# LouisBearing/BirdSoundClassif

Hardware: AMD Instinct MI355X
Metric: clips/sec (3 s @ 22.05 kHz) detect fwd (higher is better)
Workload: dtype f32; 1 GPU; BASELINE.json configs[1]: 1xMI355X inference, batch=64 synthetic 3 s clips (PCM16 @22.05 kHz resident in HBM) through the HIP STFT front end + detector forward + device post-processing, detections returned to the host; batch_per_gpu=64, distinct_clips=64, lanes=2

## Files before the change

birdsoundclassif_amd/_lib.py:

```python
import ctypes as C
import os
import subprocess

_HERE = os.path.dirname(os.path.abspath(__file__))
LIB_PATH = os.environ.get('NBM_LIB') or os.path.join(_HERE, 'libnbm_hip.so')
CSRC = os.path.join(_HERE, 'csrc')

_lib = None


class GemmDesc(C.Structure):
    _fields_ = [('x', C.c_void_p), ('w', C.c_void_p), ('y', C.c_void_p),
                ('scale', C.c_void_p), ('shift', C.c_void_p), ('residual', C.c_void_p),
                ('x_gs', C.c_int64), ('w_gs', C.c_int64), ('y_gs', C.c_int64), ('res_gs', C.c_int64),
                ('groups', C.c_int),
                ('B', C.c_int), ('H', C.c_int), ('W', C.c_int), ('Cin', C.c_int),
                ('N', C.c_int),
                ('kh', C.c_int), ('kw', C.c_int), ('stride', C.c_int), ('pad', C.c_int),
                ('Ho', C.c_int), ('Wo', C.c_int),
                ('x_ld', C.c_int), ('w_ld', C.c_int), ('y_ld', C.c_int), ('res_ld', C.c_int),
                ('alpha', C.c_float), ('act', C.c_int), ('shift_per_row', C.c_int),
                ('up', C.c_void_p), ('up_H', C.c_int), ('up_W', C.c_int),
                ('rows', C.c_void_p), ('rows_blocks', C.c_void_p),
                ('rows_mode', C.c_int), ('rows_count', C.c_int), ('rows_TH', C.c_int), ('rows_TW', C.c_int),
                ('mask', C.c_void_p), ('mask_ld', C.c_int), ('bits_out', C.c_void_p)]


class RoiDesc(C.Structure):
    _fields_ = [('fmap', C.c_void_p * 5), ('fh', C.c_int * 5), ('fw', C.c_int * 5),
                ('n_levels', C.c_int), ('C', C.c_int),
                ('rois', C.c_void_p), ('n_roi', C.c_void_p), ('B', C.c_int), ('roi_cap', C.c_int),
                ('pe_f', C.c_void_p), ('pe_t', C.c_void_p), ('img_h', C.c_int), ('img_w', C.c_int),
                ('pool', C.c_void_p), ('pe', C.c_void_p), ('level', C.c_void_p)]


class AugmentParams(C.Structure):
    _fields_ = [('gain', C.c_float), ('coef', C.c_float), ('denom', C.c_float), ('neg_coef', C.c_float),
                ('neg_denom', C.c_float), ('flags', C.c_int32), ('hard_index', C.c_int32), ('pad', C.c_int32),
                ('noise_seed', C.c_uint64)]


class BwdDesc(C.Structure):
    _fields_ = [('g', C.c_void_p), ('w', C.c_void_p), ('x', C.c_void_p), ('out', C.c_void_p),
                ('a_scale', C.c_void_p), ('row_scale', C.c_void_p), ('residual', C.c_void_p), ('mask', C.c_void_p),
                ('g_gs', C.c_int64), ('w_gs', C.c_int64), ('x_gs', C.c_int64), ('out_gs', C.c_int64), ('res_gs', C.c_int64),
                ('groups', C.c_int),
                ('B', C.c_int), ('H', C.c_int), ('W', C.c_int), ('Cin', C.c_int), ('N', C.c_int),
                ('kh', C.c_int), ('kw', C.c_int), ('stride', C.c_int), ('pad', C.c_int), ('Ho', C.c_int), ('Wo', C.c_int),
                ('g_ld', C.c_int), ('w_ld', C.c_int), ('x_ld', C.c_int), ('out_ld', C.c_int), ('res_ld', C.c_int),
                ('mask_ld', C.c_int), ('alpha', C.c_float), ('bias_grad', C.c_void_p), ('residual2', C.c_void_p), ('res2_ld', C.c_int),
                ('mask_bits', C.c_void_p)]


_P, _I, _L, _F, _U64 = C.c_void_p, C.c_int, C.c_int64, C.c_float, C.c_uint64

SIGNATURES = {
    'nbm_graph_census': [_P, C.POINTER(C.c_longlong * 6)],
    'nbm_copy_rect': [_P, _P, _L, _L, _I, _L, _L, _I, _I, _P],
    'nbm_gemm_conv': [C.POINTER(GemmDesc), _P],
    'nbm_pcm16_to_wave': [_P, _L, _I, _I, _I, _P, _L, _L, _P, _L, _I, _I, _P],
    'nbm_resample_to_wave': [_P, _L, _I, _L, _I, _I, _P, _I, _L, _L, _P, _L, _I, _I, _I, _P],
    'nbm_wav_decode': [_P, _L, _I, _I, _I, _I, _L, _P, _L, _P],
    'nbm_minmax_init': [_P, _I, _P],
    'nbm_stft_db': [_P, _L, _I, _I, _I, _I, _P, _I, _I, _I, _F, _P, _L, _I, _P, _P],
    'nbm_spec_windows': [_P, _L, _I, _I, _I, _I, _P, _P, _I, _I, _I, _P, _P],
    'nbm_spec_windows_table': [_P, _I, _I, _P, _I, _I, _P],
    'nbm_init_conv': [_P, _L, _P, _P, _I, _P, _P],
    'nbm_stem7x7': [_P, _I, _I, _I, _P, _P, _P, _P, _P, _P, _P],
    'nbm_stem7x7_wgrad': [_P, _P, _I, _I, _I, _P, _P, _P],
    'nbm_maxpool3x3s2': [_P, _I, _I, _I, _I, _P, _I, _I, _P, _P],
    'nbm_space_to_batch2': [_P, _I, _I, _I, _I, _P, _I, _P],
    'nbm_avgpool2x2': [_P, _I, _I, _I, _I, _P, _P],
    'nbm_avgpool2x2_bwd': [_P, _I, _I, _I, _I, _P, _P],
    'nbm_upsample_bilinear_add': [_P, _I, _I, _I, _I, _P, _P, _I, _I, _P],
    'nbm_softmax_rows': [_P, _L, _I, _L, _P],
    'nbm_dwconv3x3': [_P, _I, _I, _I, _I, _I, _I, _P, _P, _P, _L, _P, _I, _I, _P],
    'nbm_silu': [_P, _P, _L, _P],
    'nbm_layernorm': [_P, _L, _I, _P, _P, _F, _P, _P],
    'nbm_mha_small': [_P, _P, _P, _I, _I, _I, _P, _I, _I, _I, _I, _I, _L, _L, _P, _F, _P],
    'nbm_mha_segments': [_P, _P, _P, _I, _I, _I, _P, _I, _I, _I, _I, _I, _I, _P, _P, _I, _F, _P],
    'nbm_pair_softmax': [_P, _L, _I, _I, _P, _I, _P],
    'nbm_rpn_decode': [_P, _P, _P, _I, _I, _I, _I, _I, _I, _P, _P, _P, _P],
    'nbm_nan_images': [_P, _I, _L, _P, _P],
    'nbm_rpn_select': [_P, _P, _P, _I, _I, _I, _I, _I, _P, _P, _P, _P, _P],
    'nbm_nms_batched': [_P, _P, _P, _I, _I, _F, _I, _P, _P, _P, _P, _P, _P, _P],
    'nbm_roi_pool': [C.POINTER(RoiDesc), _P],
    'nbm_rcnn_post': [_P, _P, _I, _I, _P, _P, _I, _I, _I, _F, _F, _I, _P, _P, _P],
    'nbm_merge_collect': [_P, _P, _I, _I, _I, _I, _I, _L, _P, _P, _P, _P, _P, _P],
    'nbm_merge_nms_workspace': [_I, C.POINTER(C.c_int64)],
    'nbm_merge_nms': [_P, _P, _I, _F, _P, _L, _P, _P, _P],
    'nbm_merge_gather': [_P, _P, _P, _P, _P, _I, _P, _P, _P],
    'nbm_conv_dgrad': [C.POINTER(BwdDesc), _P],
    'nbm_conv_wgrad': [C.POINTER(BwdDesc), _P],
    'nbm_relu_bwd': [_P, _P, _P, _L, _P],
    'nbm_silu_bwd': [_P, _P, _P, _L, _P],
    'nbm_axpby': [_P, _P, _P, _F, _F, _L, _L, _P],
    'nbm_colsum': [_P, _L, _I, _I, _P, _P],
    'nbm_leaky_relu_bwd': [_P, _P, _P, _F, _L, _P],
    'nbm_layernorm_bwd': [_P, _P, _P, _L, _I, _F, _P, _P, _P, _P],
    'nbm_mha_small_bwd': [_P, _P, _P, _P, _I, _I, _I, _I, _P, _P, _P, _I, _I, _I, _P, _I, _I, _I, _I, _L, _L, _P, _F, _P],
    'nbm_zero_roi_windows': [_P, _I, _I, _I, _P, _P, _I, _I, _I, _P],
    'nbm_zero_pattern': [_P, _I, _I, _I, _I, _I, _P],
    'nbm_zero_tiles': [_P, _I, _I, _I, _I, _P, _I, _P, _P],
    'nbm_tiles_gather': [_P, _I, _I, _I, _I, _P, _I, _P, _P, _P],
    'nbm_tiles_scatter_add': [_P, _I, _I, _I, _I, _P, _I, _P, _P, _P],
    'nbm_proposal_iou': [_P, _P, _P, _I, _I, _I, _P, _P, _P],
    'nbm_anchor_targets': [_P, _I, _P, _P, _I, _I, _F, _F, _P, _P, _P, _P],
    'nbm_maxpool3x3s2_bwd': [_P, _P, _P, _I, _I, _I, _I, _I, _I, _P, _P, _P],
    'nbm_upsample_bilinear_bwd': [_P, _I, _I, _I, _I, _P, _I, _I, _I, _P],
    'nbm_tiles_upsample_bilinear_bwd_add': [_P, _I, _I, _I, _I, _P, _I, _P, _P, _I, _I, _P],
    'nbm_png_unfilter_gray8': [_P, _L, _I, _I, _I, _P, _L, _P, _P],
    'nbm_image_half_std_u8': [_P, _L, _I, _L, _P, _P],
    'nbm_randn_fill': [_U64, _L, _P, _P],
    'nbm_augment_batch': [_P, _P, _P, _I, _I, _I, _P, _P, _P, _P, _P, _P, _P],
    'nbm_u8_to_unit': [_P, _L, _P, _P],
    'nbm_wino_input': [_P, _I, _I, _I, _I, _P, _I, _P],
    'nbm_wino_output': [_P, _P, _P, _P, _I, _I, _I, _I, _I, _P, _I, _P, _P],
    'nbm_wino_outgrad': [_P, _I, _I, _I, _I, _P, _P, _I, _P],
    'nbm_wino_weight': [_P, _P, _I, _I, _I, _I, _P, _P],
    'nbm_wino_weight_grad': [_P, _P, _I, _I, _I, _P, _P],
    'nbm_wino23_rows': [_P, _I, _I, _I, _I, _P, _P],
    'nbm_wino23_conv_fused': [_P, _P, _P, _P, _P, _I, _I, _I, _I, _I, _I, _P, _I, _P],
    'nbm_wino23_rows_tiles': [_P, _I, _I, _I, _I, _P, _I, _P, _P, _P, _I, _P],
    'nbm_wino23_conv_fused_tiles': [_P, _P, _P, _P, _P, _I, _I, _I, _I, _I, _I, _P, _P, _I, _P, _P, _P],
    'nbm_roi_tiles': [_P, _P, _I, _I, _I, _I, _P, _P, _P, _I, _P, _P, _P],
    'nbm_wino23_input_tiles': [_P, _I, _I, _I, _I, _P, _I, _P, _P, _P],
    'nbm_wino23_outgrad_tiles': [_P, _I, _I, _I, _I, _P, _I, _P, _P, _P, _I, _P],
    'nbm_cell_outgrad': [_P, _I, _I, _I, _I, _I, _P, _P, _P],
    'nbm_cell_weight': [_P, _I, _I, _P, _I, _P, _I, _P],
    'nbm_cell_weight_fold': [_P, _P, _I, _I, _I, _I, _F, _P, _I, _P, _I, _P],
    'nbm_cell_weight_grad': [_P, _I, _I, _I, _P, _P],
    'nbm_cell_input': [_P, _I, _I, _I, _I, _I, _P, _I, _I, _P],
    'nbm_cell_input_up': [_P, _P, _I, _I, _I, _I, _I, _I, _I, _P, _I, _I, _P],
    'nbm_cell_patches': [_P, _I, _I, _I, _I, _I, _P, _I, _I, _P],
    'nbm_cell_patches_up': [_P, _P, _I, _I, _I, _I, _I, _I, _I, _P, _I, _I, _P],
    'nbm_cell_dgrad_output': [_P, _I, _I, _I, _I, _I, _P, _I, _I, _I, _P, _P],
    'nbm_cell_output': [_P, _P, _I, _I, _I, _I, _I, _P, _P],
    'nbm_weighted_sum': [_P, _P, _P, _P, _P, _L, _P],
    'nbm_weighted_sum_bwd': [_P, _P, _P, _P, _P, _P, _P, _P, _P, _L, _P],
    'nbm_softmax_rows_bwd': [_P, _P, _P, _L, _I, _F, _P],
    'nbm_pair_softmax_bwd': [_P, _P, _P, _L, _P],
    'nbm_dwconv3x3_bwd': [_P, _P, _P, _I, _I, _I, _I, _I, _I, _P, _P, _P, _I, _I, _P],
# ... 51 lines not shown
```

birdsoundclassif_amd/csrc/igemm.hip:

```cpp
#include <stdlib.h>
#include "nbm_common.h"
#include "igemm_params.h"
#include <type_traits>

namespace {

constexpr int BK = 32;
constexpr int PITCH = 36;

enum { A_FAST = 0, A_GENERIC = 1 };
enum { EPI_STD = 0 };

using nbm_igemm::IgemmParams;

template <int BM, int BN, int WM, int WN, int AMODE, int EPI, int STAGES = 2, bool ROWS = false>
__global__ __launch_bounds__(256, BM > 128 ? 1 : STAGES == 1 ? 3 : 2) void igemm_kernel(const IgemmParams p) {
  constexpr int MT = WM / 32, NT = WN / 32;
  constexpr int WAVES_N = BN / WN;
  constexpr int AR = BM / 32, BR = BN / 32;
  static_assert((BM / WM) * (BN / WN) == 4, "4 waves per workgroup");

  __shared__ __attribute__((aligned(16))) float lds[STAGES * (BM + BN) * PITCH];
  if constexpr (STAGES == 2) nbm_stagger_priority();
  float* As = lds;
// ... 319 lines not shown
#pragma unroll
        for (int j = 0; j < NTG; ++j) {
          const float* wb = Ws + ((g * NTG + j) * 32 + li) * WP + 16 * lh;
#pragma unroll
          for (int kc = 0; kc < K32; ++kc) {
            f32x4 b[4];
#pragma unroll
            for (int q = 0; q < 4; ++q) b[q] = *reinterpret_cast<const f32x4*>(wb + kc * 32 + 4 * q);
#pragma unroll
            for (int q = 0; q < 4; ++q)
#pragma unroll
              for (int e = 0; e < 4; ++e) acc[j] = __builtin_amdgcn_mfma_f32_32x32x2f32(a[kc][q][e], b[q][e], acc[j], 0, 0, 0);
          }
        }
      }
#pragma unroll
      for (int j = 0; j < NTG; ++j) {
        const int jj = g * NTG + j;
        __builtin_amdgcn_fence(__ATOMIC_ACQ_REL, "wavefront");
#pragma unroll
        for (int e = 0; e < 16; ++e) stg[((e & 3) + 8 * (e >> 2) + 4 * lh) * SPITCH + li] = acc[j][e];
        __builtin_amdgcn_fence(__ATOMIC_ACQ_REL, "wavefront");
        const int n = n_off + jj * 32 + ec;
        f32x4 sc = {1.f, 1.f, 1.f, 1.f}, sh = {0.f, 0.f, 0.f, 0.f};
        if (p.scale) sc = *reinterpret_cast<const f32x4*>(p.scale + n);
        if (p.shift) sh = *reinterpret_cast<const f32x4*>(p.shift + n);
#pragma unroll
        for (int pass = 0; pass < 4; ++pass) {
          const int r = pass * 8 + er, m = m0 + r;
          if (m >= p.M) continue;
          f32x4 v = *reinterpret_cast<const f32x4*>(stg + r * SPITCH + ec);
#pragma unroll
          for (int e = 0; e < 4; ++e) v[e] = (v[e] * p.alpha) * sc[e] + sh[e] + 0.f;
          if (p.residual) { v[0] += rq[j][pass][0]; v[1] += rq[j][pass][1]; v[2] += rq[j][pass][2]; v[3] += rq[j][pass][3]; }
          if (p.act == NBM_ACT_RELU) {
#pragma unroll
            for (int e = 0; e < 4; ++e) v[e] = fmaxf(v[e], 0.0f);
          } else if (p.act == NBM_ACT_SILU) {
#pragma unroll
            for (int e = 0; e < 4; ++e) v[e] = v[e] / (1.0f + expf(-v[e]));
          } else if (p.act == NBM_ACT_LEAKY) {
#pragma unroll
            for (int e = 0; e < 4; ++e) v[e] = v[e] > 0.f ? v[e] : 0.01f * v[e];
          }
          if (p.bits_out) {
            const int grp8 = 8 * er;
            const unsigned wb = ((unsigned)(__builtin_amdgcn_ballot_w64(v[0] > 0.f) >> grp8) & 0xffu) |
                                (((unsigned)(__builtin_amdgcn_ballot_w64(v[1] > 0.f) >> grp8) & 0xffu) << 8) |
                                (((unsigned)(__builtin_amdgcn_ballot_w64(v[2] > 0.f) >> grp8) & 0xffu) << 16) |
                                (((unsigned)(__builtin_amdgcn_ballot_w64(v[3] > 0.f) >> grp8) & 0xffu) << 24);
            if (ec == 0) Bw[wave][r * NT + jj] = wb;
          }
          *reinterpret_cast<f32x4*>(p.y + (long long)m * p.y_ld + n) = v;
        }
      }
    }
    if (p.bits_out) {
      static_assert(NT >= 2 && NT % 2 == 0, "two lanes per tile row");
      constexpr int WPL = NT / 2;
      __builtin_amdgcn_fence(__ATOMIC_ACQ_REL, "wavefront");
      const int r = lane >> 1, j0 = (lane & 1) * WPL;
      const int m = m0 + r;
      if (m < p.M) {
        unsigned* dst = p.bits_out + (long long)m * p.n_words + (n_off >> 5) + j0;
        const unsigned* src = Bw[wave] + r * NT + j0;
        if constexpr (WPL == 4) *reinterpret_cast<uint4*>(dst) = *reinterpret_cast<const uint4*>(src);
        else if constexpr (WPL == 2) *reinterpret_cast<uint2*>(dst) = *reinterpret_cast<const uint2*>(src);
        else {
#pragma unroll
          for (int q = 0; q < WPL; ++q) dst[q] = src[q];
        }
      }
      __builtin_amdgcn_fence(__ATOMIC_ACQ_REL, "wavefront");
    }
  }
}

template <int K32, int NT, int NTG, int WAVES, int WG_PER_CU>
int launch_stream(const StreamParams& p, hipStream_t st, int slices = 1) {
  const int wgs = (p.m_tiles + WAVES - 1) / WAVES;
  int gx = 256 * WG_PER_CU / slices;
  if (gx < 1) gx = 1;
  hipLaunchKernelGGL((stream1x1_kernel<K32, NT, NTG, WAVES>), dim3(wgs < gx ? wgs : gx, slices), dim3(WAVES * 64), 0, st, p);
  return nbm_launch_status();
}

template <int BM, int BN, int WM, int WN, int AMODE, int EPI>
int launch(const IgemmParams& p, int groups, hipStream_t st) {
  dim3 grid(p.m_tiles * p.n_tiles, 1, groups);
  hipLaunchKernelGGL((igemm_kernel<BM, BN, WM, WN, AMODE, EPI>), grid, dim3(256), 0, st, p);
  return nbm_launch_status();
}

int launch_s1(const IgemmParams& p, int groups, hipStream_t st) {
  dim3 grid(p.m_tiles * p.n_tiles, 1, groups);
  hipLaunchKernelGGL((igemm_kernel<128, 128, 64, 64, A_FAST, EPI_STD, 1>), grid, dim3(256), 0, st, p);
  return nbm_launch_status();
}

int launch_s1_rows(const IgemmParams& p, hipStream_t st) {
  const int mt = p.rows_blocks ? (p.m_tiles + 7) / 8 * 8 : p.m_tiles;
  dim3 grid(mt * p.n_tiles, 1, 1);
  hipLaunchKernelGGL((igemm_kernel<128, 128, 64, 64, A_FAST, EPI_STD, 1, true>), grid, dim3(256), 0, st, p);
  return nbm_launch_status();
}

}

extern "C" int nbm_gemm_conv(const nbm_gemm_desc* d, void* stream) {
  if (!d || !d->x || !d->w || !d->y) return NBM_EINVAL;
  if (d->B <= 0 || d->H <= 0 || d->W <= 0 || d->Cin <= 0 || d->N <= 0 || d->kh <= 0 || d->kw <= 0 ||
      d->stride <= 0 || d->Ho <= 0 || d->Wo <= 0 || d->groups <= 0)
    return NBM_EINVAL;
  if ((d->H + 2 * d->pad - d->kh) / d->stride + 1 != d->Ho || (d->W + 2 * d->pad - d->kw) / d->stride + 1 != d->Wo)
    return NBM_EINVAL;
  if (d->x_ld < d->Cin || d->y_ld < d->N || (d->residual && d->res_ld < d->N)) return NBM_EINVAL;
  if (d->N > 128 && (d->N & 127) == 64 && !d->rows && !d->up && !d->bits_out && !d->shift_per_row && (d->Cin % BK) == 0 &&
      d->kh * d->kw * d->Cin > 256) {
    nbm_gemm_desc a = *d, b = *d;
    const int n0 = d->N - 64;
    a.N = n0;
    b.N = 64;
    b.w = d->w + (long long)n0 * d->w_ld;
    b.y = d->y + n0;
    if (d->scale) b.scale = d->scale + n0;
    if (d->shift) b.shift = d->shift + n0;
    if (d->residual) b.residual = d->residual + n0;
    if (d->mask) b.mask = d->mask + n0;
    const int rc = nbm_gemm_conv(&a, stream);
    return rc ? rc : nbm_gemm_conv(&b, stream);
  }
  IgemmParams p{};
  p.x = d->x; p.w = d->w; p.y = d->y; p.scale = d->scale; p.shift = d->shift; p.residual = d->residual;
  p.x_gs = d->x_gs; p.w_gs = d->w_gs; p.y_gs = d->y_gs; p.res_gs = d->res_gs;
  p.M = d->B * d->Ho * d->Wo; p.N = d->N; p.K = d->kh * d->kw * d->Cin;
  p.nk = (p.K + BK - 1) / BK;
  p.H = d->H; p.W = d->W; p.Cin = d->Cin; p.kh = d->kh; p.kw = d->kw; p.stride = d->stride; p.pad = d->pad;
  p.Ho = d->Ho; p.Wo = d->Wo; p.HoWo = d->Ho * d->Wo;
  p.fd_howo = nbm_fastdiv_make((unsigned)p.HoWo); p.fd_wo = nbm_fastdiv_make((unsigned)p.Wo);
  p.x_ld = d->x_ld; p.w_ld = d->w_ld; p.y_ld = d->y_ld; p.res_ld = d->res_ld;
  p.alpha = d->alpha; p.act = d->act; p.shift_per_row = d->shift_per_row;
  if (p.w_ld < p.nk * BK) return NBM_EINVAL;
  if (d->mask) {
    if (d->rows || d->groups != 1 || d->mask_ld < d->N) return NBM_EUNSUPPORTED;
    p.mask = d->mask; p.mask_ld = d->mask_ld;
  }
  p.vec_epi = ((d->N & 3) == 0 && (d->y_ld & 3) == 0 && (d->y_gs & 3) == 0 && nbm_aligned16(d->y) &&
               (!d->residual || ((d->res_ld & 3) == 0 && (d->res_gs & 3) == 0 && nbm_aligned16(d->residual))) &&
               (!d->scale || nbm_aligned16(d->scale)) && (!d->shift || d->shift_per_row || nbm_aligned16(d->shift)) &&
               (!d->mask || ((d->mask_ld & 3) == 0 && nbm_aligned16(d->mask))))
                  ? 1 : 0;
  if ((d->w_ld & 3) || (d->w_gs & 3) || !nbm_aligned16(d->w)) return NBM_EALIGN;
  if (d->bits_out) {
    if (!p.vec_epi || (d->N & 31) || d->groups != 1 || d->rows) return NBM_EUNSUPPORTED;
    p.bits_out = d->bits_out;
  }
  if (d->up) {
    if (!p.vec_epi || d->groups != 1 || d->up_H <= 0 || d->up_W <= 0 || !nbm_aligned16(d->up)) return NBM_EUNSUPPORTED;
    p.up = d->up; p.up_H = d->up_H; p.up_W = d->up_W;
    p.up_sh = d->Ho > 1 ? (float)(d->up_H - 1) / (float)(d->Ho - 1) : 0.f;
    p.up_sw = d->Wo > 1 ? (float)(d->up_W - 1) / (float)(d->Wo - 1) : 0.f;
  }
  const bool fast = (d->Cin % BK) == 0 && (d->x_ld & 3) == 0 && (d->x_gs & 3) == 0 && nbm_aligned16(d->x);
  hipStream_t st = (hipStream_t)stream;
  const int BM = 128;
  p.m_tiles = (p.M + BM - 1) / BM;
  if (d->rows) {
    if (d->kh != 1 || d->kw != 1 || d->stride != 1 || d->pad != 0 || d->groups != 1 || !fast || !p.vec_epi || d->shift_per_row ||
        p.nk > 8 || d->N <= 64 || (d->rows_mode != 1 && d->rows_mode != 2) || d->rows_count <= 0 || (d->rows_count % 128))
      return NBM_EUNSUPPORTED;
    if (d->rows_mode == 2 && (d->rows_TH != (d->H + 1) / 2 || d->rows_TW != (d->W + 1) / 2)) return NBM_EINVAL;
    if (2ll * d->H * d->W * d->x_ld * 4 > 0x7fffffffll) return NBM_EUNSUPPORTED;
    p.rows = d->rows; p.rows_blocks = d->rows_blocks; p.rows_mode = d->rows_mode; p.rows_TH = d->rows_TH; p.rows_TW = d->rows_TW;
    p.fd_rows_thw = nbm_fastdiv_make((unsigned)(d->rows_TH * d->rows_TW)); p.fd_rows_tw = nbm_fastdiv_make((unsigned)d->rows_TW);
    p.M = d->rows_count;
    p.m_tiles = p.M / BM;
    p.n_tiles = (d->N + 127) / 128;
    return launch_s1_rows(p, st);
  }
  const char* stream_env = getenv("NBM_STREAM1X1");
  if (!(stream_env && stream_env[0] == '0') && d->kh == 1 && d->kw == 1 && d->stride == 1 && d->pad == 0 && d->groups == 1 && fast && p.vec_epi && !d->up && !d->mask &&
      !d->shift_per_row && (d->N % 32) == 0 && p.M >= 8192) {
    StreamParams sp{d->x, d->w, d->y, d->scale, d->shift, d->residual, p.M, d->x_ld, d->w_ld, d->y_ld, d->res_ld, (p.M + 31) / 32,
                    d->alpha, d->act, d->bits_out, d->N >> 5};
    const int k32 = d->Cin / 32, nt = d->N / 32;
    if (k32 == 2 && nt == 8 && d->residual) return launch_stream<2, 8, 4, 8, 1>(sp, st);
    if (k32 == 2 && nt == 2) return launch_stream<2, 2, 2, 8, 2>(sp, st);
    if (k32 == 8 && nt == 2) return launch_stream<8, 2, 2, 8, 1>(sp, st);
    if (d->residual) {
      if (k32 == 4 && nt % 4 == 0 && nt <= 32) return launch_stream<4, 4, 4, 8, 1>(sp, st, nt / 4);
      if (k32 == 8 && nt % 2 == 0 && nt <= 64) return launch_stream<8, 2, 2, 8, 1>(sp, st, nt / 2);
    }
  }
  if (d->N > 64) {
    p.n_tiles = (d->N + 127) / 128;
    const char* split_env = getenv("NBM_SPLIT_BF16");
    if (split_env && split_env[0] == '1' && fast && p.vec_epi && p.nk >= 9 && d->kh * d->kw < 63)
      return nbm_igemm::split_launch(p, d->groups, st);
    const char* h16_env = getenv("NBM_H16");
    if (!(h16_env && atoi(h16_env) == 0) && fast && p.vec_epi && p.nk >= 9 && d->kh * d->kw < 63) return nbm_igemm::h16_launch(p, d->groups, st);
    if (fast && p.vec_epi && p.nk <= 8)
      return launch_s1(p, d->groups, st);

    return fast ? launch<128, 128, 64, 64, A_FAST, EPI_STD>(p, d->groups, st)
                : launch<128, 128, 64, 64, A_GENERIC, EPI_STD>(p, d->groups, st);
  } else if (d->N > 32) {
    p.n_tiles = 1;
    if (fast && p.vec_epi && p.nk <= 20) {
      dim3 grid(p.m_tiles * p.n_tiles, 1, d->groups);
      hipLaunchKernelGGL((igemm_kernel<128, 64, 64, 32, A_FAST, EPI_STD, 1>), grid, dim3(256), 0, st, p);
      return nbm_launch_status();
    }
    return fast ? launch<128, 64, 64, 32, A_FAST, EPI_STD>(p, d->groups, st)
                : launch<128, 64, 64, 32, A_GENERIC, EPI_STD>(p, d->groups, st);
  } else {
    p.n_tiles = 1;
    return fast ? launch<128, 32, 32, 32, A_FAST, EPI_STD>(p, d->groups, st)
                : launch<128, 32, 32, 32, A_GENERIC, EPI_STD>(p, d->groups, st);
  }
}
```

birdsoundclassif_amd/nets/backbone.py:

```python
import torch
from torch import nn

from .. import ops
from . import _prep, functional as Fn
from .position_encoding import build_position_encoding

bcbk_channels = {'resnet': {'2': 64, '3': 256, '4': 512, '5': 1024, '6': 2048}}
_RESNET_LAYERS = {'resnet50': [3, 4, 6, 3], 'resnet101': [3, 4, 23, 3], 'resnet152': [3, 8, 36, 3]}


class FrozenBatchNorm2d(nn.Module):

    def __init__(self, n):
        super().__init__()
        self.register_buffer('weight', torch.ones(n))
        self.register_buffer('bias', torch.zeros(n))
        self.register_buffer('running_mean', torch.zeros(n))
        self.register_buffer('running_var', torch.ones(n))

    def _load_from_state_dict(self, state_dict, prefix, local_metadata, strict, missing_keys, unexpected_keys,
                              error_msgs):
        state_dict.pop(prefix + 'num_batches_tracked', None)
        super()._load_from_state_dict(state_dict, prefix, local_metadata, strict, missing_keys, unexpected_keys,
                                      error_msgs)

    def affine(self):
        return _prep.bn_affine(self.weight, self.bias, self.running_mean, self.running_var, 1e-5, frozen=True)


class _Bottleneck(nn.Module):

    def __init__(self, inplanes, planes, stride, downsample, norm_layer):
        super().__init__()
        self.conv1 = nn.Conv2d(inplanes, planes, 1, bias=False)
        self.bn1 = norm_layer(planes)
        self.conv2 = nn.Conv2d(planes, planes, 3, stride=stride, padding=1, bias=False)
        self.bn2 = norm_layer(planes)
        self.conv3 = nn.Conv2d(planes, planes * 4, 1, bias=False)
        self.bn3 = norm_layer(planes * 4)
        self.downsample = downsample
        self.stride = stride
        self.mask_input, self.mask_gy = False, True

    def forward(self, x):
        if torch.is_grad_enabled() and x.dim() == 4 and self.conv1.weight.shape[0] % 32 == 0:
            ds = self.downsample
            sd, bd = ds[1].affine() if ds is not None else (None, None)
            return Fn.Bottleneck.apply(x, self.conv1.weight, self.conv2.weight, self.conv3.weight,
                                       ds[0].weight if ds is not None else None, *self.bn1.affine(), *self.bn2.affine(),
                                       *self.bn3.affine(), sd, bd, self.stride, self.mask_input, self.mask_gy)
        s, b = self.bn1.affine()
        o = Fn.conv(x, self.conv1.weight, scale=s, shift=b, act=ops.ACT_RELU)
        s, b = self.bn2.affine()
        if self.stride == 1 and Fn._winograd_ok(o, self.conv2.weight, 3, 3, 1, 1):
            o = ops.conv3x3_winograd(o, _prep.wino23(self.conv2.weight), b, scale=s, relu=True)
        else:
            o = Fn.conv(o, self.conv2.weight, scale=s, shift=b, kh=3, kw=3, stride=self.stride, pad=1, act=ops.ACT_RELU)
        if self.downsample is not None:
            s, b = self.downsample[1].affine()
            idt = Fn.conv(x, self.downsample[0].weight, scale=s, shift=b, stride=self.stride)
        else:
            idt = x
        s, b = self.bn3.affine()
        return Fn.conv(o, self.conv3.weight, scale=s, shift=b, residual=idt, act=ops.ACT_RELU)


class _ResNetBody(nn.Module):

    def __init__(self, layers, norm_layer, dilation=False):
        super().__init__()
        self.conv1 = nn.Conv2d(3, 64, 7, stride=2, padding=3, bias=False)
        self.bn1 = norm_layer(64)
        self.dilation = bool(dilation)
        inplanes = 64
        for li, (planes, n, stride) in enumerate(zip((64, 128, 256, 512), layers, (1, 2, 2, 1 if dilation else 2)), start=1):
            blocks = []
            for bi in range(n):
                st = stride if bi == 0 else 1
                ds = None
                if bi == 0 and (st != 1 or inplanes != planes * 4):
                    ds = nn.Sequential(nn.Conv2d(inplanes, planes * 4, 1, stride=st, bias=False), norm_layer(planes * 4))
                blocks.append(_Bottleneck(inplanes, planes, st, ds, norm_layer))
                if dilation and li == 4 and bi > 0:
                    blocks[-1].conv2.dilation, blocks[-1].conv2.padding = (2, 2), (2, 2)
                blocks[-1].mask_input = not (li == 1 and bi == 0)
                blocks[-1].mask_gy = bi == n - 1
                inplanes = planes * 4
            setattr(self, f'layer{li}', nn.Sequential(*blocks))

    def forward(self, x, init_conv=None):
        s, b = self.bn1.affine()
        if init_conv is not None:
            x = Fn.Stem.apply(x, init_conv.weight, init_conv.bias, self.conv1.weight, s, b)
        else:
            x = Fn.conv(x, self.conv1.weight, scale=s, shift=b, kh=7, kw=7, stride=2, pad=3, act=ops.ACT_RELU)
        taps = [x]
        x = Fn.MaxPool.apply(x, True)
        for li in range(1, 5):
            for bi, blk in enumerate(getattr(self, f'layer{li}')):
                if self.dilation and li == 4 and bi == 1:
                    x = Fn.SpaceToBatch2.apply(x, False)
                x = blk(x)
            if self.dilation and li == 4 and len(self.layer4) > 1:
                x = Fn.SpaceToBatch2.apply(x, True)
            taps.append(x)
        return taps


class BackboneBase(nn.Module):

    def __init__(self, backbone, name, in_channels, train_backbone):
        super().__init__()
        for _, parameter in backbone.named_parameters():
            if not train_backbone:
                parameter.requires_grad_(False)
        self.body = backbone
        self.num_channels = list(bcbk_channels['resnet'].values())
        if in_channels != 3:
            self.init_conv = nn.Conv2d(in_channels, 3, 1)
        self.in_channels = in_channels
        self.strides = [2 ** (i + 1) for i in range(len(self.num_channels))]

    def forward(self, x):
        if hasattr(self, 'init_conv'):
            if self.in_channels != 1:
                raise NotImplementedError('init_conv is implemented for 1 input channel (reference default)')
            return self.body(x, self.init_conv)
        return self.body(x)


class Backbone(BackboneBase):

    def __init__(self, name, in_channels, train_backbone, dilation, norm_layer_name):
        if name not in _RESNET_LAYERS:
            raise ValueError(f'not supported {name}: the accelerated path implements {sorted(_RESNET_LAYERS)}')
        if norm_layer_name != 'frozen_batchnorm':
            raise NotImplementedError('only --norm_layer_backbone frozen_batchnorm (reference default) is implemented')
        super().__init__(_ResNetBody(_RESNET_LAYERS[name], FrozenBatchNorm2d, dilation=dilation), name, in_channels, train_backbone)


# ... 18 lines not shown
```

birdsoundclassif_amd/ops.py:

```python
import ctypes as C
import os
import math

import torch

from . import _lib
from ._lib import GemmDesc, RoiDesc, check

ACT_NONE, ACT_RELU, ACT_SILU, ACT_LEAKY = 0, 1, 2, 3

PROFILE = None
FLOPS = None
FLOPS_DEFERRED = []


def flops_total():
    tot = FLOPS[0] + sum(float(c.item()) * f for c, f in FLOPS_DEFERRED)
    FLOPS_DEFERRED.clear()
    return tot


_PROFILE_LABEL = None
PROFILE_ONLY = None

# ... 21 lines not shown

def _chk(t, dtype=torch.float32, name='tensor'):
    if not (isinstance(t, torch.Tensor) and t.is_cuda):
        raise RuntimeError(f'{name}: the NBM HIP path needs CUDA (ROCm) tensors; no CPU fallback exists')
    if t.dtype != dtype:
        raise TypeError(f'{name}: expected {dtype}, got {t.dtype}')
    if not t.is_contiguous():
        raise ValueError(f'{name}: must be contiguous')
    return t


def lib():
    return _lib.load()


def gemm_conv(x, w, y, *, B, H, W, Cin, N, kh=1, kw=1, stride=1, pad=0, Ho=None, Wo=None,
              x_ld=None, w_ld=None, y_ld=None, scale=None, shift=None, residual=None, res_ld=None,
              groups=1, x_gs=0, w_gs=0, y_gs=0, res_gs=0, alpha=1.0, act=ACT_NONE, shift_per_row=False, up=None,
              rows=None, rows_mode=0, rows_count=0, rows_blocks=None, rows_thw=(0, 0), mask=None, mask_ld=None, bits_out=None):
    Ho = (H + 2 * pad - kh) // stride + 1 if Ho is None else Ho
    Wo = (W + 2 * pad - kw) // stride + 1 if Wo is None else Wo
    d = GemmDesc()
    d.x, d.w, d.y = x.data_ptr(), w.data_ptr(), y.data_ptr()
    d.scale = scale.data_ptr() if scale is not None else None
    d.shift = shift.data_ptr() if shift is not None else None
    d.residual = residual.data_ptr() if residual is not None else None
    d.x_gs, d.w_gs, d.y_gs, d.res_gs = x_gs, w_gs, y_gs, res_gs
    d.groups = groups
    d.B, d.H, d.W, d.Cin, d.N = B, H, W, Cin, N
    d.kh, d.kw, d.stride, d.pad, d.Ho, d.Wo = kh, kw, stride, pad, Ho, Wo
    d.x_ld = Cin if x_ld is None else x_ld
    d.w_ld = kh * kw * Cin if w_ld is None else w_ld
    d.y_ld = N if y_ld is None else y_ld
    d.res_ld = (N if res_ld is None else res_ld) if residual is not None else 0
    d.alpha, d.act, d.shift_per_row = float(alpha), int(act), int(bool(shift_per_row))
    if up is not None:
        d.up, d.up_H, d.up_W = _chk(up, name='up').data_ptr(), up.shape[1], up.shape[2]
    if mask is not None:
        d.mask, d.mask_ld = mask.data_ptr(), int(N if mask_ld is None else mask_ld)
    if bits_out is not None:
        assert bits_out.dtype == torch.int32 and bits_out.is_contiguous() and bits_out.numel() * 32 >= B * Ho * Wo * N and N % 32 == 0
        d.bits_out = bits_out.data_ptr()
    if rows is not None:
        d.rows, d.rows_mode, d.rows_count = rows.data_ptr(), int(rows_mode), int(rows_count)
        d.rows_blocks = rows_blocks.data_ptr() if rows_blocks is not None else None
        d.rows_TH, d.rows_TW = rows_thw
    if FLOPS is not None:
        if rows is None:
            FLOPS[0] += 2.0 * B * Ho * Wo * N * kh * kw * Cin * groups
        elif rows_blocks is None:
            FLOPS[0] += 2.0 * rows_count * N * Cin
        else:
            FLOPS_DEFERRED.append((rows_blocks.clone(), 2.0 * 128 * (16 if rows_mode == 2 else 1) * N * Cin))
    if _prof_all() or (PROFILE is not None and PROFILE_ONLY == 'deepk' and is_deepk(Cin, N, kh, kw, rows)):
        ev0, ev1 = torch.cuda.Event(enable_timing=True), torch.cuda.Event(enable_timing=True)
        ev0.record()
        check(lib().nbm_gemm_conv(C.byref(d), _stream()), 'nbm_gemm_conv')
        ev1.record()
        if rows is None:
            PROFILE.append(((Cin, N, kh, H, W, B, groups, stride, _PROFILE_LABEL), ev0, ev1))
        elif rows_blocks is None:
            PROFILE.append(((Cin, N, kh, rows_count, 1, 1, groups, stride, ('rows', H, W)), ev0, ev1))
        else:
            PROFILE.append(((Cin, N, kh, 0, 1, 1, groups, stride, ('rows-rois', H, W)), ev0, ev1))
        return y
    check(lib().nbm_gemm_conv(C.byref(d), _stream()), 'nbm_gemm_conv')
    return y


def conv2d(x, w, kh=1, kw=1, stride=1, pad=0, scale=None, shift=None, residual=None, act=ACT_NONE,
           alpha=1.0, out=None, w_ld=None, up=None, bits_out=None):
    _chk(x, name='x'), _chk(w, name='w')
    B, H, W, Cin = x.shape
    N = w.shape[0]
    Ho = (H + 2 * pad - kh) // stride + 1
    Wo = (W + 2 * pad - kw) // stride + 1
    y = out if out is not None else torch.empty((B, Ho, Wo, N), device=x.device, dtype=torch.float32)
    if residual is not None:
        _chk(residual, name='residual')
        assert residual.shape == y.shape
    gemm_conv(x, w, y, B=B, H=H, W=W, Cin=Cin, N=N, kh=kh, kw=kw, stride=stride, pad=pad, Ho=Ho, Wo=Wo,
              w_ld=w.shape[1] if w_ld is None else w_ld, scale=scale, shift=shift, residual=residual,
              alpha=alpha, act=act, up=up, bits_out=bits_out)
    return y


WINO_CHUNK_BYTES = 24 << 30
_WINO_SCRATCH = {}

LANE = 0


class lane:
    def __init__(self, k):
        self.k = int(k)

    def __enter__(self):
        global LANE
        self.prev, LANE = LANE, self.k

    def __exit__(self, *exc):
        global LANE
        LANE = self.prev


def _wino_scratch(device, n_v, n_m):
    need = n_v + n_m
    key = (device, LANE)
    buf = _WINO_SCRATCH.get(key)
    if buf is None or buf.numel() < need:
        if torch.cuda.is_current_stream_capturing():
            raise RuntimeError('the persistent Winograd scratch would have to grow during a graph capture (the warm-up steps of the '
                               'capture must run the same shapes under the same ops.lane)')
        have = 0 if buf is None else buf.numel()
        _WINO_SCRATCH[key] = buf = None
        size = min(max(need, 2 * have), max(need, WINO_CHUNK_BYTES // 4))
        buf = _WINO_SCRATCH[key] = torch.empty((size,), device=device, dtype=torch.float32)
    return buf[:n_v], buf[n_v:need]


GRAPH_NODE_KINDS = ('kernel', 'memcpy', 'memset', 'host', 'empty', 'other')


def graph_census(raw_graph):
    counts = (C.c_longlong * 6)()
    check(_lib.load().nbm_graph_census(C.c_void_p(int(raw_graph)), C.byref(counts)), 'nbm_graph_census')
    return dict(zip(GRAPH_NODE_KINDS, (int(v) for v in counts)))


def lane_buffers(lanes):
    from . import ondemand
    held = [buf for key, buf in _WINO_SCRATCH.items() if key[1] in lanes and buf is not None]
    for key, bufs in ondemand._ROI_TILE_BUF.items():
        if key[2] in lanes:
            held.extend(bufs)
    return held


def release_lane_scratch(keep=(0,)):
    from . import ondemand
    for key in [k for k in _WINO_SCRATCH if k[1] not in keep]:
        del _WINO_SCRATCH[key]
    for key in [k for k in ondemand._ROI_TILE_BUF if k[2] not in keep]:
        del ondemand._ROI_TILE_BUF[key]


def conv3x3_winograd(x, U, bias=None, m=2, scale=None, relu=False, mask=None, residual=None):
    _chk(x, name='x'), _chk(U, name='U')
    B, H, W, C_ = x.shape
    N = U.shape[1]
    nxi = (m + 2) ** 2
    assert U.shape == (nxi, N, C_) and C_ % 32 == 0 and N % 4 == 0
    y = torch.empty((B, H, W, N), device=x.device, dtype=torch.float32)
    tiles = (-(-H // m)) * (-(-W // m))
    fused = m == 2 and C_ >= 64
    assert residual is None or m == 4, 'residual: F(4x4,3x3) output transform only' 
    if fused:
        per_img = 4 * (-(-H // 2)) * (2 * (-(-W // 2)) + 2) * C_ * 4
    else:
        per_img = nxi * tiles * (C_ + N) * 4
    chunk = max(1, min(B, WINO_CHUNK_BYTES // per_img))
    if fused:
        V, M = _wino_scratch(x.device, chunk * per_img // 4, 0)
    else:
        V, M = _wino_scratch(x.device, nxi * chunk * tiles * C_, nxi * chunk * tiles * N)
    st = _stream()
# ... 964 lines not shown
```

include/nbm_hip.h:

```cpp
#ifndef NBM_HIP_H
#define NBM_HIP_H

#include <stdint.h>

#ifdef __cplusplus
extern "C" {
#endif

#define NBM_OK 0
#define NBM_EINVAL (-1)
#define NBM_EALIGN (-2)
#define NBM_EUNSUPPORTED (-3)

#define NBM_ACT_NONE 0
#define NBM_ACT_RELU 1
#define NBM_ACT_SILU 2
#define NBM_ACT_LEAKY 3

const char* nbm_version(void);

int nbm_graph_census(void* graph, long long counts[6]);

typedef struct nbm_gemm_desc {
  const float* x;
  const float* w;
  float* y;
  const float* scale;
  const float* shift;
  const float* residual;
  int64_t x_gs, w_gs, y_gs, res_gs;
  int groups;
  int B, H, W, Cin;
  int N;
  int kh, kw, stride, pad;
  int Ho, Wo;
  int x_ld, w_ld, y_ld, res_ld;
  float alpha;
  int act;
  int shift_per_row;
  const float* up;
  int up_H, up_W;
  const int* rows;
  const int* rows_blocks;
  int rows_mode, rows_count, rows_TH, rows_TW;
  const float* mask;
  int mask_ld;
  unsigned* bits_out;
} nbm_gemm_desc;

int nbm_gemm_conv(const nbm_gemm_desc* d, void* stream);

int nbm_wino_input(const float* x, int B, int H, int W, int C, float* V, int m, void* stream);
int nbm_wino_output(const float* M, const float* scale, const float* shift, const float* mask, int relu, int B, int H, int W,
                    int N, float* y, int m, const float* residual, void* stream);
int nbm_wino_outgrad(const float* g, int B, int H, int W, int N, float* dM, float* bias_grad, int m, void* stream);

int nbm_wino_weight(const float* g, const float* scale, int N, int C, int transposed, int m, float* U, void* stream);
int nbm_wino_weight_grad(const float* dU, const float* row_scale, int N, int C, int m, float* dW, void* stream);

int nbm_wino23_rows(const float* x, int B, int H, int W, int C, float* R, void* stream);
int nbm_wino23_conv_fused(const float* R, const float* U, const float* scale, const float* shift, const float* mask,
                          int relu, int B, int H, int W, int C, int N, float* y, int variant, void* stream);

int nbm_wino23_rows_tiles(const float* x, int B, int H, int W, int C, const int* tiles, int n_entries, const int* n_blocks,
                          const unsigned* blk_info, float* R,
                          int skip_pattern_stride ,
                          void* stream);
int nbm_wino23_conv_fused_tiles(const float* R, const float* U, const float* scale, const float* shift, const float* mask,
                                int relu ,
                                int B, int H, int W, int C, int N, float* y, const int* tiles, int n_entries,
                                const int* n_blocks, const unsigned* blk_info, void* stream);
int nbm_roi_tiles(const float* rois, const int* n_roi, int B, int roi_cap, int n_levels, int level, const int* fh,
                  const int* fw, const unsigned char* skip, int dilate, int* tiles, int* n_blocks, void* stream);
int nbm_wino23_input_tiles(const float* x, int B, int H, int W, int C, const int* tiles, int n_list, const unsigned* plane_mask,
                           float* V, void* stream);
int nbm_wino23_outgrad_tiles(const float* g, int B, int H, int W, int N, const int* tiles, int n_list, const unsigned* plane_mask,
                             float* dM, float* bias_grad, int skip_pattern_stride, void* stream);
int nbm_cell_outgrad(const float* g, int B, int H, int W, int N, int stride, float* Vg, float* bias_grad, void* stream);
int nbm_cell_weight(const float* w, int N, int C, float* U_nc, int ld, float* U_cn, int ldt, void* stream);
int nbm_cell_weight_fold(const float* w, const float* w_lat, int wl_ld, int N, int C, int Cin, float alpha, float* U_nc, int ld,
                         float* U_cn, int ldt, void* stream);
int nbm_cell_weight_grad(const float* dU, int N, int C, int ld, float* dW, void* stream);
int nbm_cell_input(const float* x, int B, int H, int W, int C, int stride, float* Vx, int ld ,
                   int c_off , void* stream);
int nbm_cell_input_up(const float* x1, const float* bias, int B, int H, int W, int C, int Hc, int Wc, int stride, float* Vx, int ld,
                      int c_off, void* stream);
int nbm_cell_patches(const float* x, int B, int H, int W, int C, int stride, float* Vx, int ld, int c_off, void* stream);
int nbm_cell_patches_up(const float* x1, const float* bias, int B, int H, int W, int C, int Hc, int Wc, int stride, float* Vx, int ld,
                        int c_off, void* stream);

int nbm_copy_rect(float* strided, float* packed, int64_t n_outer, int64_t outer_pitch, int n_rows, int64_t row_pitch, int64_t width,
                  int to_strided, int zero_strided, void* stream);
int nbm_cell_dgrad_output(const float* M, int B, int H, int W, int C, int stride, float* gx, int parity_class,
                          int ld , int c_off ,
                          float* bias_grad , void* stream);
int nbm_cell_output(const float* M, const float* bias, int B, int H, int W, int N, int stride, float* y, void* stream);


int nbm_pcm16_to_wave(const int16_t* pcm, int64_t pcm_ld, int batch, int n, int upsample,
                      const int32_t* hq, int64_t first, int64_t count, float* out, int64_t out_ld, int lead,
                      int pad_mode, void* stream);

int nbm_resample_to_wave(const float* x, int64_t x_ld, int batch, int64_t n, int L, int M, const double* taps, int T,
                         int64_t first, int64_t count, float* out, int64_t out_ld, int lead, int pad_mode, int quant16,
                         void* stream);

#define NBM_WAV_MAX_CHANNELS 8
int nbm_wav_decode(const void* raw, int64_t raw_pitch, int batch, int tag, int bits, int channels, int64_t n, float* out,
                   int64_t out_pitch, void* stream);

int nbm_minmax_init(uint32_t* minmax, int batch, void* stream);
int nbm_stft_db(const float* wave, int64_t wave_ld, int batch, int n_frames, int hop, int n_fft,
                const double* basis, int basis_bin_tiles, int basis_ksteps, int n_bins, float floor_amp,
                float* db, int64_t db_bs, int db_ld, uint32_t* minmax, void* stream);

int nbm_spec_windows(const float* db, int64_t db_bs, int db_ld, int batch, int n_bins, int n_frames,
                     const uint32_t* minmax, float* img, int n_img, int w_pix, int hop_img,
                     const int32_t* last_cols, void* stream);

typedef struct nbm_window_entry {
  const float* db;
  const uint32_t* minmax;
  const int32_t* last_cols;
  int32_t db_ld, n_frames, window, n_img;
} nbm_window_entry;

int nbm_spec_windows_table(const nbm_window_entry* table, int batch, int n_bins, float* img, int w_pix, int hop_img,
                           void* stream);


int nbm_init_conv(const float* x, int64_t n_pix, const float* w, const float* b, int C, float* y, void* stream);

int nbm_stem7x7(const float* img, int B, int H, int W, const float* weff, const float* wb, const float* wb_full,
// ... 183 lines not shown
```

Measured before the change: 1060 clips/s.

## Fuse bottleneck conv3 and downsample 1x1 convs into one dual-GEMM kernel

Adds a HIP kernel that computes the ResNet bottleneck's final 1x1 conv and the downsample 1x1 conv together, applying both BN affines, the residual add and the ReLU in one pass. It is used for stride-1 blocks with 64 input channels and 256 output channels, i.e. the first block of layer1. This removes the intermediate identity tensor write and re-read and one kernel launch. The cost is extra LDS use and one-WG-per-CU launch bounds, which may reduce occupancy compared with the tuned generic path.

```diff
diff --git a/birdsoundclassif_amd/_lib.py b/birdsoundclassif_amd/_lib.py
--- a/birdsoundclassif_amd/_lib.py
+++ b/birdsoundclassif_amd/_lib.py
@@ -58,6 +58,7 @@
     'nbm_graph_census': [_P, C.POINTER(C.c_longlong * 6)],
     'nbm_copy_rect': [_P, _P, _L, _L, _I, _L, _L, _I, _I, _P],
     'nbm_gemm_conv': [C.POINTER(GemmDesc), _P],
+    'nbm_conv1x1_dual': [_P, _I, _P, _I, _P, _P, _F, _P, _I, _P, _I, _P, _P, _P, _I, _I, _P],
     'nbm_pcm16_to_wave': [_P, _L, _I, _I, _I, _P, _L, _L, _P, _L, _I, _I, _P],
     'nbm_resample_to_wave': [_P, _L, _I, _L, _I, _I, _P, _I, _L, _L, _P, _L, _I, _I, _I, _P],
     'nbm_wav_decode': [_P, _L, _I, _I, _I, _I, _L, _P, _L, _P],
diff --git a/birdsoundclassif_amd/csrc/igemm.hip b/birdsoundclassif_amd/csrc/igemm.hip
--- a/birdsoundclassif_amd/csrc/igemm.hip
+++ b/birdsoundclassif_amd/csrc/igemm.hip
@@ -425,6 +425,119 @@
   int gx = 256 * WG_PER_CU / slices;
   if (gx < 1) gx = 1;
   hipLaunchKernelGGL((stream1x1_kernel<K32, NT, NTG, WAVES>), dim3(wgs < gx ? wgs : gx, slices), dim3(WAVES * 64), 0, st, p);
+  return nbm_launch_status();
+}
+
+struct DualParams {
+  const float* a; const float* wa; const float* sca; const float* sha;
+  const float* x; const float* wb; const float* scb; const float* shb;
+  float* y;
+  int M, a_ld, wa_ld, x_ld, wb_ld, y_ld, m_tiles; float alpha_a, alpha_b;
+};
+
+#define NBM_EPI_AFFINE(t, sc, sh) __builtin_fmaf((t), (sc), (sh))
+template <int NT, int WAVES>
+__global__ __launch_bounds__(WAVES * 64, 1) void stream1x1_dual_kernel(const DualParams p) {
+#pragma clang fp contract(off)
+  constexpr int K = 64, N = NT * 32, WP = K + 4;
+  __shared__ __attribute__((aligned(16))) float Wa[N * WP];
+  __shared__ __attribute__((aligned(16))) float Wb[N * WP];
+  __shared__ __attribute__((aligned(16))) float Stg[WAVES][32 * SPITCH];
+  __shared__ float Aff[4][N];
+  const int tid = threadIdx.x, lane = tid & 63, wave = tid >> 6, li = lane & 31, lh = lane >> 5;
+  const int n_off = blockIdx.y * N;
+  for (int i = tid; i < N * (K / 4); i += WAVES * 64) {
+    const int n = i / (K / 4), c = i - n * (K / 4);
+    *reinterpret_cast<f32x4*>(Wa + n * WP + c * 4) = *reinterpret_cast<const f32x4*>(p.wa + (long long)(n_off + n) * p.wa_ld + c * 4);
+    *reinterpret_cast<f32x4*>(Wb + n * WP + c * 4) = *reinterpret_cast<const f32x4*>(p.wb + (long long)(n_off + n) * p.wb_ld + c * 4);
+  }
+  for (int n = tid; n < N; n += WAVES * 64) {
+    Aff[0][n] = p.sca ? p.sca[n_off + n] : 1.f;
+    Aff[1][n] = p.sha ? p.sha[n_off + n] : 0.f;
+    Aff[2][n] = p.scb ? p.scb[n_off + n] : 1.f;
+    Aff[3][n] = p.shb ? p.shb[n_off + n] : 0.f;
+  }
+  __syncthreads();
+  float* stg = Stg[wave];
+  const int er = lane >> 3, ec = (lane & 7) * 4;
+  f32x4 a[2][4], x[2][4], an[2][4], xn[2][4];
+  auto row_of = [&](int tile) {
+    const int m = tile * 32 + li;
+    return (long long)(m < p.M ? m : p.M - 1);
+  };
+  auto load_rows = [&](const float* rp, f32x4 (*dst)[4]) {
+#pragma unroll
+    for (int kc = 0; kc < 2; ++kc)
+#pragma unroll
+      for (int q = 0; q < 4; ++q) dst[kc][q] = *reinterpret_cast<const f32x4*>(rp + kc * 32 + 4 * q);
+  };
+  const int step = gridDim.x * WAVES;
+  int tile = blockIdx.x * WAVES + wave;
+  if (tile < p.m_tiles) {
+    const long long m = row_of(tile);
+    load_rows(p.a + m * p.a_ld + 16 * lh, an);
+    load_rows(p.x + m * p.x_ld + 16 * lh, xn);
+  }
+  for (; tile < p.m_tiles; tile += step) {
+    const long long mn = row_of(tile + step < p.m_tiles ? tile + step : tile);
+#pragma unroll
+    for (int kc = 0; kc < 2; ++kc)
+#pragma unroll
+      for (int q = 0; q < 4; ++q) { a[kc][q] = an[kc][q]; x[kc][q] = xn[kc][q]; }
+    load_rows(p.a + mn * p.a_ld + 16 * lh, an);
+    load_rows(p.x + mn * p.x_ld + 16 * lh, xn);
+    const int m0 = tile * 32;
+#pragma unroll
+    for (int j = 0; j < NT; ++j) {
+      f32x16 acca, accb;
+#pragma unroll
+      for (int e = 0; e < 16; ++e) { acca[e] = 0.f; accb[e] = 0.f; }
+      const float* wa = Wa + (j * 32 + li) * WP + 16 * lh;
+      const float* wb = Wb + (j * 32 + li) * WP + 16 * lh;
+#pragma unroll
+      for (int kc = 0; kc < 2; ++kc) {
+        f32x4 ba[4], bb[4];
+#pragma unroll
+        for (int q = 0; q < 4; ++q) {
+          ba[q] = *reinterpret_cast<const f32x4*>(wa + kc * 32 + 4 * q);
+          bb[q] = *reinterpret_cast<const f32x4*>(wb + kc * 32 + 4 * q);
+        }
+#pragma unroll
+        for (int q = 0; q < 4; ++q)
+#pragma unroll
+          for (int e = 0; e < 4; ++e) {
+            acca = __builtin_amdgcn_mfma_f32_32x32x2f32(a[kc][q][e], ba[q][e], acca, 0, 0, 0);
+            accb = __builtin_amdgcn_mfma_f32_32x32x2f32(x[kc][q][e], bb[q][e], accb, 0, 0, 0);
+          }
+      }
+      const int nl = j * 32 + li;
+      const float sa = Aff[0][nl], ha = Aff[1][nl], sb = Aff[2][nl], hb = Aff[3][nl];
+      __builtin_amdgcn_fence(__ATOMIC_ACQ_REL, "wavefront");
+#pragma unroll
+      for (int e = 0; e < 16; ++e) {
+        const float idt = NBM_EPI_AFFINE(accb[e] * p.alpha_b, sb, hb) + 0.f;
+        float v = NBM_EPI_AFFINE(acca[e] * p.alpha_a, sa, ha) + 0.f;
+        v += idt;
+        stg[((e & 3) + 8 * (e >> 2) + 4 * lh) * SPITCH + li] = fmaxf(v, 0.0f);
+      }
+      __builtin_amdgcn_fence(__ATOMIC_ACQ_REL, "wavefront");
+      const int n = n_off + j * 32 + ec;
+#pragma unroll
+      for (int pass = 0; pass < 4; ++pass) {
+        const int r = pass * 8 + er, m = m0 + r;
+        if (m >= p.M) continue;
+        *reinterpret_cast<f32x4*>(p.y + (long long)m * p.y_ld + n) = *reinterpret_cast<const f32x4*>(stg + r * SPITCH + ec);
+      }
+    }
+  }
+}
+
+template <int NT, int WAVES>
+int launch_dual(const DualParams& p, hipStream_t st) {
+  constexpr int slices = 8 / NT;
+  const int wgs = (p.m_tiles + WAVES - 1) / WAVES;
+  const int gx = 256 / slices;
+  hipLaunchKernelGGL((stream1x1_dual_kernel<NT, WAVES>), dim3(wgs < gx ? wgs : gx, slices), dim3(WAVES * 64), 0, st, p);
   return nbm_launch_status();
 }
 
@@ -562,3 +675,15 @@
                 : launch<128, 32, 32, 32, A_GENERIC, EPI_STD>(p, d->groups, st);
   }
 }
+
+extern "C" int nbm_conv1x1_dual(const float* a, int a_ld, const float* wa, int wa_ld, const float* scale_a, const float* shift_a, float alpha,
+                                const float* x, int x_ld, const float* wb, int wb_ld, const float* scale_b, const float* shift_b,
+                                float* y, int y_ld, int M, void* stream) {
+  if (!a || !wa || !x || !wb || !y || M <= 0) return NBM_EINVAL;
+  if (a_ld < 64 || x_ld < 64 || wa_ld < 64 || wb_ld < 64 || y_ld < 256) return NBM_EINVAL;
+  if (((a_ld | x_ld | wa_ld | wb_ld | y_ld) & 3) || !nbm_aligned16(a) || !nbm_aligned16(x) || !nbm_aligned16(wa) || !nbm_aligned16(wb) ||
+      !nbm_aligned16(y))
+    return NBM_EALIGN;
+  DualParams p{a, wa, scale_a, shift_a, x, wb, scale_b, shift_b, y, M, a_ld, wa_ld, x_ld, wb_ld, y_ld, (M + 31) / 32, alpha, 1.0f};
+  return launch_dual<4, 8>(p, (hipStream_t)stream);
+}
diff --git a/birdsoundclassif_amd/nets/backbone.py b/birdsoundclassif_amd/nets/backbone.py
--- a/birdsoundclassif_amd/nets/backbone.py
+++ b/birdsoundclassif_amd/nets/backbone.py
@@ -56,6 +56,11 @@
             o = ops.conv3x3_winograd(o, _prep.wino23(self.conv2.weight), b, scale=s, relu=True)
         else:
             o = Fn.conv(o, self.conv2.weight, scale=s, shift=b, kh=3, kw=3, stride=self.stride, pad=1, act=ops.ACT_RELU)
+        if self.downsample is not None and self.stride == 1 and not torch.is_grad_enabled() and x.dim() == 4 and \
+                x.shape[-1] == 64 and self.conv3.weight.shape[:2] == (256, 64):
+            sd, bd = self.downsample[1].affine()
+            s, b = self.bn3.affine()
+            return ops.conv1x1_dual(o, _prep.krsc(self.conv3.weight), x, _prep.krsc(self.downsample[0].weight), s, b, sd, bd)
         if self.downsample is not None:
             s, b = self.downsample[1].affine()
             idt = Fn.conv(x, self.downsample[0].weight, scale=s, shift=b, stride=self.stride)
diff --git a/birdsoundclassif_amd/ops.py b/birdsoundclassif_amd/ops.py
--- a/birdsoundclassif_amd/ops.py
+++ b/birdsoundclassif_amd/ops.py
@@ -127,6 +127,38 @@
     gemm_conv(x, w, y, B=B, H=H, W=W, Cin=Cin, N=N, kh=kh, kw=kw, stride=stride, pad=pad, Ho=Ho, Wo=Wo,
               w_ld=w.shape[1] if w_ld is None else w_ld, scale=scale, shift=shift, residual=residual,
               alpha=alpha, act=act, up=up, bits_out=bits_out)
+    return y
+
+
+def conv1x1_dual(a, wa, x, wb, scale_a=None, shift_a=None, scale_b=None, shift_b=None, alpha=1.0):
+    _chk(a, name='a'), _chk(x, name='x'), _chk(wa, name='wa'), _chk(wb, name='wb')
+    B, H, W, Ca = a.shape
+    if not (x.shape == a.shape and Ca == 64 and wa.shape[0] == 256 and wb.shape[0] == 256 and wa.shape[1] >= 64 and wb.shape[1] >= 64):
+        raise ValueError(f'conv1x1_dual: two [B,H,W,64] maps and two [256, >= 64] weight matrices, got {tuple(a.shape)}, '
+                         f'{tuple(x.shape)}, {tuple(wa.shape)}, {tuple(wb.shape)}')
+    M = B * H * W
+    fused = os.environ.get('NBM_DUAL1X1') != '0' and os.environ.get('NBM_STREAM1X1', '1')[:1] != '0' and M >= 8192 and \
+        wa.shape[1] % 4 == 0 and wb.shape[1] % 4 == 0 and \
+        all(t is None or t.data_ptr() % 16 == 0 for t in (a, x, wa, wb, scale_a, shift_a, scale_b, shift_b))
+    if not fused:
+        idt = conv2d(x, wb, scale=scale_b, shift=shift_b)
+        return conv2d(a, wa, scale=scale_a, shift=shift_a, residual=idt, act=ACT_RELU, alpha=alpha)
+    for t, name in ((scale_a, 'scale_a'), (shift_a, 'shift_a'), (scale_b, 'scale_b'), (shift_b, 'shift_b')):
+        if t is not None:
+            assert _chk(t, name=name).numel() == 256
+    y = torch.empty((B, H, W, 256), device=a.device, dtype=torch.float32)
+    if FLOPS is not None:
+        FLOPS[0] += 2.0 * M * 256 * 128
+    prof = _prof_all()
+    if prof:
+        ev = (torch.cuda.Event(enable_timing=True), torch.cuda.Event(enable_timing=True))
+        ev[0].record()
+    check(lib().nbm_conv1x1_dual(_ptr(a), 64, _ptr(wa), wa.shape[1], _ptr(scale_a), _ptr(shift_a), float(alpha),
+                                 _ptr(x), 64, _ptr(wb), wb.shape[1], _ptr(scale_b), _ptr(shift_b), _ptr(y), 256, M, _stream()),
+          'nbm_conv1x1_dual')
+    if prof:
+        ev[1].record()
+        PROFILE.append(((128, 256, 1, H, W, B, 1, 1, None), *ev))
     return y
 
 
diff --git a/include/nbm_hip.h b/include/nbm_hip.h
--- a/include/nbm_hip.h
+++ b/include/nbm_hip.h
@@ -49,6 +49,10 @@
 } nbm_gemm_desc;
 
 int nbm_gemm_conv(const nbm_gemm_desc* d, void* stream);
+
+int nbm_conv1x1_dual(const float* a, int a_ld, const float* wa, int wa_ld, const float* scale_a, const float* shift_a, float alpha,
+                     const float* x, int x_ld, const float* wb, int wb_ld, const float* scale_b, const float* shift_b,
+                     float* y, int y_ld, int M, void* stream);
 
 int nbm_wino_input(const float* x, int B, int H, int W, int C, float* V, int m, void* stream);
 int nbm_wino_output(const float* M, const float* scale, const float* shift, const float* mask, int relu, int B, int H, int W,
```

Measured after the change: 1067 clips/s (median of 6 runs). About the same (+0.6%).
